# felipemcoelho/nf4-triton-dequantization

Hardware: AMD Instinct MI355X
Metric: dequantized elements/s (4096x4096 NF4->bf16, blocksize 64 / nested 256) (higher is better)
Workload: dtype f32

## Files before the change

nf4_triton_dequantization_amd/csrc/nf4_dequant.hip:

```cpp
#include <hip/hip_runtime.h>
#include <stdint.h>

#include "../../include/nf4_dequant.h"
#include "nf4_common.h"

namespace {

using namespace nf4dq;

enum Mode : int { kRef = 0, kSingle = 1, kBnb = 2, kBnbSingle = 3 };

struct Desc {
    const uint32_t* packed;
    const uint8_t* a1;
    const float* a2;
    const float* code2;
    u32x4* out;
    float offset;
    uint32_t nbytes;
    uint32_t tile_begin;
    uint32_t groups;
    FastDiv nb;
    FastDiv n2;
    FastDiv bpr;
    uint32_t blk_shift;
    uint32_t blk2_shift;
    uint32_t blk_base;
};

#ifndef NF4_FLAT_STAMPS
#define NF4_FLAT_STAMPS 0
#endif

template <int MAXB>
struct Batch {
    Desc d[MAXB];
    uint32_t count;
    uint32_t total_tiles;
#if NF4_FLAT_STAMPS
    unsigned long long* stamps;
#endif
};

#if NF4_FLAT_STAMPS
#define NF4_FSTAMP(slot_, val_)                                                                      \
    do {                                                                                             \
        __builtin_amdgcn_sched_barrier(0);                                                           \
        if (lane == 0) bt.stamps[(blockIdx.x * kFlatWaves + (threadIdx.x >> 6)) * 4u + (slot_)] = (val_); \
        __builtin_amdgcn_sched_barrier(0);                                                           \
    } while (0)
#define NF4_FNOW() __builtin_amdgcn_s_memrealtime()
#else
#define NF4_FSTAMP(slot_, val_) \
    do {                        \
    } while (0)
#define NF4_FNOW() 0ull
#endif

template <int DT>
__device__ __forceinline__ void store1(void* out, int64_t i, float x) {
    if constexpr (DT == NF4DQ_BF16) {
        reinterpret_cast<__bf16*>(out)[i] = (__bf16)x;
    } else if constexpr (DT == NF4DQ_F16) {
        reinterpret_cast<_Float16*>(out)[i] = (_Float16)opaque(x);
    } else {
        reinterpret_cast<float*>(out)[i] = x;
    }
}

#ifndef NF4_DQ_FLAT_WAVES
#define NF4_DQ_FLAT_WAVES 4
#endif
#ifndef NF4_DQ_U
#define NF4_DQ_U 4
#endif
#ifndef NF4_DQ_AUX_STORE
#define NF4_DQ_AUX_STORE 18
#endif
#ifndef NF4_DQ_AUX_LOAD
#define NF4_DQ_AUX_LOAD 2
#endif
#ifndef NF4_DQ_SCALE_FIRST
#define NF4_DQ_SCALE_FIRST 0
#endif
#ifndef NF4_DQ_SCALE_NT
#define NF4_DQ_SCALE_NT 0
#endif
#ifndef NF4_DQ_DECODE
#define NF4_DQ_DECODE 1
#endif
#ifndef NF4_DQ_SINGLE_FAST
#define NF4_DQ_SINGLE_FAST 1
#endif
#ifndef NF4_DQ_ABL_NOSCALE
#define NF4_DQ_ABL_NOSCALE 0
#endif



constexpr int kWg = 256;
constexpr int kFlatWaves = NF4_DQ_FLAT_WAVES;
constexpr int kFlatWg = 64 * kFlatWaves;
constexpr int kU = NF4_DQ_U;

constexpr int kAuxStore = NF4_DQ_AUX_STORE;
constexpr int kAuxLoad = NF4_DQ_AUX_LOAD;

template <int DT>
constexpr uint32_t out_bytes_per_packed_byte() { return DT == NF4DQ_F32 ? 8u : 4u; }
template <int DT>
constexpr uint32_t lane_bytes() { return DT == NF4DQ_F32 ? 2u : 4u; }
template <int DT>
constexpr uint32_t tile_bytes() { return 64u * lane_bytes<DT>() * kU; }

struct TileIn {
    uint32_t w[kU];
    uint32_t a1;
    float a2;
};

template <int DT>
__device__ __forceinline__ uint32_t tile_block(const Desc& D, uint32_t base, uint32_t lane) {
    constexpr uint32_t kTileBytes = tile_bytes<DT>();
    const uint32_t bsh = D.blk_shift;
    const uint32_t bpt = kTileBytes >> bsh;
    uint32_t g = (base >> bsh) + (bpt ? (lane & (bpt - 1u)) : 0u);
    const uint32_t nblk = (D.nbytes + (1u << bsh) - 1u) >> bsh;
    g = g < nblk ? g : nblk - 1u;
    return g + D.blk_base;
}

template <int DT, int MODE>
__device__ __forceinline__ TileIn tile_load(const Desc& D, __amdgpu_buffer_rsrc_t rp, uint32_t base, uint32_t lane) {
    constexpr uint32_t LB = lane_bytes<DT>();
    TileIn in;
    auto packed_loads = [&]() {
#pragma unroll
        for (int j = 0; j < kU; ++j) {
            const uint32_t off = base + 64u * LB * j + LB * lane;
            if constexpr (LB == 4) {
                in.w[j] = __builtin_amdgcn_raw_buffer_load_b32(rp, off, 0, kAuxLoad);
            } else {
                in.w[j] = __builtin_amdgcn_raw_buffer_load_b16(rp, off, 0, kAuxLoad);
            }
        }
    };
    if constexpr (!NF4_DQ_SCALE_FIRST) packed_loads();
    const uint32_t g = tile_block<DT>(D, base, lane);
    if constexpr (NF4_DQ_ABL_NOSCALE) {
        in.a1 = g & 255u;
        in.a2 = 0.01f;
    } else if constexpr (MODE == kRef) {
        const uint32_t r = fdiv(g, D.bpr);
        const uint32_t b = g - r * D.bpr.d;
        const uint8_t* pa1 = D.a1 + fmodu(g, D.nb);
        const float* pa2 = D.a2 + fmodu(r * D.groups + (b >> 2), D.n2);
        if constexpr (NF4_DQ_SCALE_NT) {
            in.a1 = __builtin_nontemporal_load(pa1);
            in.a2 = __builtin_nontemporal_load(pa2);
        } else {
            in.a1 = *pa1;
            in.a2 = *pa2;
        }
    } else if constexpr (MODE == kSingle) {
        const uint32_t r = fdiv(g, D.bpr);
        const uint32_t b = g - r * D.bpr.d;
        in.a2 = D.a2[r * D.n2.d + b];
    } else if constexpr (MODE == kBnb) {
        in.a1 = D.a1[g];
        in.a2 = D.a2[g >> D.blk2_shift];
    } else {
        in.a2 = D.a2[g];
    }
    if constexpr (NF4_DQ_SCALE_FIRST) packed_loads();
    return in;
}

template <int DT, int MODE>
__device__ __forceinline__ void tile_finish(const Desc& D, __amdgpu_buffer_rsrc_t ro, const float* lut,
                                            const TileIn& in, uint32_t base, uint32_t lane, const float* code2s) {
    float s;
    if constexpr (MODE == kRef) {
        s = ((float)in.a1 / 127.0f) * in.a2;
    } else if constexpr (MODE == kBnb) {
        s = code2s[in.a1] * in.a2 + D.offset;
    } else {
        s = in.a2;
    }
    const uint32_t bsh = D.blk_shift;
    constexpr uint32_t kOB = out_bytes_per_packed_byte<DT>();
    constexpr uint32_t LB = lane_bytes<DT>();
#pragma unroll
    for (int j = 0; j < kU; ++j) {
        const uint32_t rel = 64u * LB * j + LB * lane;
        const float sj = __shfl(s, (int)(rel >> bsh), 64);
        const uint32_t w = in.w[j];
        const uint32_t hi4 = (w >> 2) & 0x3C3C3C3Cu;
        const uint32_t lo4 = (w << 2) & 0x3C3C3C3Cu;
        const char* t = reinterpret_cast<const char*>(lut);
        float v[2 * LB];
#pragma unroll
        for (int k = 0; k < (int)LB; ++k) {
            v[2 * k] = *reinterpret_cast<const float*>(t + ((hi4 >> (8 * k)) & 0xFFu)) * sj;
            v[2 * k + 1] = *reinterpret_cast<const float*>(t + ((lo4 >> (8 * k)) & 0xFFu)) * sj;
        }
        const uint32_t ob = (base + rel) * kOB;
        if constexpr (DT == NF4DQ_F32) {
            u32x4 o = {__float_as_uint(v[0]), __float_as_uint(v[1]), __float_as_uint(v[2]), __float_as_uint(v[3])};
            __builtin_amdgcn_raw_buffer_store_b128(o, ro, ob, 0, kAuxStore);
        } else {
            u32x4 o = {pack2<DT>(v[0], v[1]), pack2<DT>(v[2], v[3]), pack2<DT>(v[4], v[5]), pack2<DT>(v[6], v[7])};
            __builtin_amdgcn_raw_buffer_store_b128(o, ro, ob, 0, kAuxStore);
        }
    }
}

typedef uint16_t __attribute__((may_alias)) u16_alias;
typedef uint32_t __attribute__((may_alias)) u32_alias;
typedef uint32_t u32x4_alias __attribute__((ext_vector_type(4), may_alias));

struct TblCtx {
    char* tbl;
    uint32_t tb;
    f32x2 c01;
};

template <int DT, int MODE>
__device__ __forceinline__ void tile_finish_tbl(const Desc& D, __amdgpu_buffer_rsrc_t ro, const TileIn& in,
                                                uint32_t base, uint32_t lane, const float* code2s,
                                                const TblCtx& c) {
    float s;
    if constexpr (MODE == kRef) {
        s = ((float)in.a1 / 127.0f) * in.a2;
    } else if constexpr (MODE == kBnb) {
        s = code2s[in.a1] * in.a2 + D.offset;
    } else {
        s = in.a2;
    }
    const uint32_t bsh = D.blk_shift;
    const uint32_t k = lane & 7u;
#pragma unroll
    for (int j = 0; j < kU; ++j) {
        const uint32_t rel = 256u * j + 4u * lane;
        const float sj = __shfl(s, (int)(rel >> bsh), 64);
        *reinterpret_cast<u32_alias*>(c.tbl + c.tb + 4u * k) = pack2<DT>(c.c01.x * sj, c.c01.y * sj);
        const uint32_t w = in.w[j];
        const uint32_t hb = (w >> 3) & 0x1E1E1E1Eu;
        const uint32_t lb = (w << 1) & 0x1E1E1E1Eu;
        uint32_t o[4];
#pragma unroll
        for (int b = 0; b < 4; ++b) {
            const uint32_t ah = __builtin_amdgcn_perm(hb, c.tb, 0x03020104u + b);
            const uint32_t al = __builtin_amdgcn_perm(lb, c.tb, 0x03020104u + b);
            const uint32_t vh = *reinterpret_cast<const u16_alias*>(c.tbl + ah);
            const uint32_t vl = *reinterpret_cast<const u16_alias*>(c.tbl + al);
            o[b] = vh | (vl << 16);
        }
        const u32x4 ov = {o[0], o[1], o[2], o[3]};
        __builtin_amdgcn_raw_buffer_store_b128(ov, ro, (base + rel) * 4u, 0, kAuxStore);
    }
}

template <int MAXB>
__device__ __forceinline__ uint32_t find_matrix(const Batch<MAXB>& bt, uint32_t t, uint32_t k) {
    if constexpr (MAXB > 1) {
        while (k + 1 < bt.count && t >= bt.d[k + 1].tile_begin) ++k;
    }
    return k;
}

struct Cursor {
    uint32_t t, k, base;
    bool valid;
};

template <int DT, int MAXB>
__device__ __forceinline__ Cursor cursor_at(const Batch<MAXB>& bt, uint32_t t, uint32_t k_hint) {
    constexpr uint32_t kTileBytes = tile_bytes<DT>();
    Cursor c;
    c.t = t;
    c.valid = t < bt.total_tiles;
    c.k = c.valid ? find_matrix(bt, t, k_hint) : k_hint;
    c.base = c.valid ? (t - bt.d[c.k].tile_begin) * kTileBytes : 0xFFFFF000u;
    return c;
}

template <int DT, int MAXB>
__device__ __forceinline__ void make_rsrcs(const Batch<MAXB>& bt, uint32_t k, __amdgpu_buffer_rsrc_t& rp,
                                           __amdgpu_buffer_rsrc_t& ro) {
    constexpr uint32_t kOB = out_bytes_per_packed_byte<DT>();
    rp = __builtin_amdgcn_make_buffer_rsrc((void*)bt.d[k].packed, 0, bt.d[k].nbytes, kRsrcFlags);
    ro = __builtin_amdgcn_make_buffer_rsrc((void*)bt.d[k].out, 0, bt.d[k].nbytes * kOB, kRsrcFlags);
}

template <int DT, int MODE, int MAXB>
__global__ __launch_bounds__(kFlatWg) void nf4_flat_kernel(const Batch<MAXB> bt) {
    __shared__ __attribute__((aligned(16))) float lut[16];
    __shared__ __attribute__((aligned(16))) float code2s[MODE == kBnb ? 256 : 1];
    constexpr bool kTbl = NF4_DQ_DECODE == 1 && DT != NF4DQ_F32;
    __shared__ __attribute__((aligned(256))) char tbl[kTbl ? kFlatWaves * 2048 : 4];
    const uint32_t lane = threadIdx.x & 63u;
#if NF4_FLAT_STAMPS
    const unsigned long long t_entry = NF4_FNOW();
    unsigned long long tiles_done = 0;
#endif
    const uint32_t t0 = __builtin_amdgcn_readfirstlane(blockIdx.x * kFlatWaves + (threadIdx.x >> 6));
    const uint32_t nwaves = gridDim.x * kFlatWaves;

    float c2w = 0.0f;
    if constexpr (MODE == kBnb) c2w = bt.d[0].code2[threadIdx.x & 255u];
    Cursor ca = cursor_at<DT>(bt, t0, 0u);
    __amdgpu_buffer_rsrc_t rpa, roa;
    make_rsrcs<DT>(bt, ca.k, rpa, roa);
    TileIn A = tile_load<DT, MODE>(bt.d[ca.k], rpa, ca.base, lane);
    const bool multi = !NF4_DQ_SINGLE_FAST || ca.t + nwaves < bt.total_tiles;
    if (multi) {
        const u32x4 z = {0u, 0u, 0u, 0u};
#pragma unroll
        for (int j = 0; j < kU; ++j) __builtin_amdgcn_raw_buffer_store_b128(z, roa, 0xFFFFF000u + 16u * j, 0, kAuxStore);
    }
    write_lut(lut);
    if constexpr (MODE == kBnb) {
        if constexpr (kFlatWg >= 256) {
            if (threadIdx.x < 256u) code2s[threadIdx.x] = c2w;
        } else {
            for (uint32_t i = threadIdx.x; i < 256u; i += kFlatWg) code2s[i] = bt.d[0].code2[i];
        }
    }
    __syncthreads();
    TblCtx tc{};
    if constexpr (kTbl) {
        tc.tbl = tbl;
        tc.tb = ((threadIdx.x >> 6) << 11) + ((lane >> 3) << 8);
        tc.c01 = *reinterpret_cast<const f32x2*>(lut + 2u * (lane & 7u));
    }
    if (!ca.valid) {
        NF4_FSTAMP(0, t_entry);
        NF4_FSTAMP(1, 0ull);
        NF4_FSTAMP(2, NF4_FNOW());
        NF4_FSTAMP(3, 0ull);
        return;
    }
    if (!multi) {
        if constexpr (kTbl) tile_finish_tbl<DT, MODE>(bt.d[ca.k], roa, A, ca.base, lane, code2s, tc);
        else tile_finish<DT, MODE>(bt.d[ca.k], roa, lut, A, ca.base, lane, code2s);
#if NF4_FLAT_STAMPS
        NF4_FSTAMP(1, NF4_FNOW());
        __builtin_amdgcn_s_waitcnt(0);
        NF4_FSTAMP(0, t_entry);
        NF4_FSTAMP(2, NF4_FNOW());
        NF4_FSTAMP(3, 1ull);
#endif
        return;
    }
    while (true) {
        const Cursor cb = cursor_at<DT>(bt, ca.t + nwaves, ca.k);
        __amdgpu_buffer_rsrc_t rpb = rpa, rob = roa;
        if (MAXB > 1 && cb.k != ca.k) make_rsrcs<DT>(bt, cb.k, rpb, rob);
        TileIn B = tile_load<DT, MODE>(bt.d[cb.k], rpb, cb.base, lane);
        if constexpr (kTbl) tile_finish_tbl<DT, MODE>(bt.d[ca.k], roa, A, ca.base, lane, code2s, tc);
        else tile_finish<DT, MODE>(bt.d[ca.k], roa, lut, A, ca.base, lane, code2s);
#if NF4_FLAT_STAMPS
        if (tiles_done == 0) NF4_FSTAMP(1, NF4_FNOW());
        ++tiles_done;
#endif
        if (!cb.valid) break;

        const Cursor cn = cursor_at<DT>(bt, cb.t + nwaves, cb.k);
        __amdgpu_buffer_rsrc_t rpn = rpb, ron = rob;
        if (MAXB > 1 && cn.k != cb.k) make_rsrcs<DT>(bt, cn.k, rpn, ron);
        A = tile_load<DT, MODE>(bt.d[cn.k], rpn, cn.base, lane);
        if constexpr (kTbl) tile_finish_tbl<DT, MODE>(bt.d[cb.k], rob, B, cb.base, lane, code2s, tc);
        else tile_finish<DT, MODE>(bt.d[cb.k], rob, lut, B, cb.base, lane, code2s);
#if NF4_FLAT_STAMPS
        ++tiles_done;
#endif
        if (!cn.valid) break;
        ca = cn;
        rpa = rpn;
        roa = ron;
    }
#if NF4_FLAT_STAMPS
    __builtin_amdgcn_s_waitcnt(0);
    NF4_FSTAMP(0, t_entry);
    NF4_FSTAMP(2, NF4_FNOW());
    NF4_FSTAMP(3, tiles_done);
#endif
}

struct RowsArgs {
    const uint8_t* packed;
    const uint8_t* a1;
    const float* a2;
    void* out;
    int64_t m, n, stride, cols_b;
    int64_t nb, n2, bpr, groups, rs;
};

template <int DT, int MODE>
__global__ __launch_bounds__(kWg) void nf4_rows_kernel(const RowsArgs A) {
    __shared__ __attribute__((aligned(16))) float lut[16];
    write_lut(lut);
    __syncthreads();
    const int64_t total = A.m * A.cols_b;
    for (int64_t i = (int64_t)blockIdx.x * kWg + threadIdx.x; i < total; i += (int64_t)gridDim.x * kWg) {
        const int64_t r = i / A.cols_b;
        const int64_t j = i - r * A.cols_b;
        const int64_t b = j >> 5;
        float s;
        if constexpr (MODE == kRef) {
            const float q = (float)A.a1[(r * A.bpr + b) % A.nb];
            s = (q / 127.0f) * A.a2[(r * A.groups + (b >> 2)) % A.n2];
        } else {
            s = A.a2[r * A.rs + b];
        }
        const uint32_t byte = A.packed[r * A.stride + j];
        const int64_t c = 2 * j;
        store1<DT>(A.out, r * A.n + c, lut[byte >> 4] * s);
        if (c + 1 < A.n) store1<DT>(A.out, r * A.n + c + 1, lut[byte & 15u] * s);
    }
}

struct ChunkArgs {
    const uint8_t* packed;
    const uint8_t* a1;
    const float* a2;
    void* out;
    uint64_t packed_len;
    uint64_t out_elems;
    uint32_t stride;
    uint32_t n;
    uint32_t chunks;
    FastDiv L;
    FastDiv bpr;
    uint32_t groups;
    FastDiv nb, n2;
    uint32_t rs;
};

constexpr uint32_t kDrop = 0xFFFFFFF0u;
constexpr int kAuxPiece = 0;
constexpr uint32_t kStageBytes = 4128;
constexpr uint32_t kStageDummy = 4112;

inline __device__ uint32_t range32(uint64_t v) { return v > 0x7FFFFFFFull ? 0x7FFFFFFFu : (uint32_t)v; }

inline __device__ uint32_t opaque_mul(uint32_t a, uint32_t b) {
    uint32_t r = a * b;
    asm("" : "+v"(r));
    return r;
}

template <int DT>
__device__ __forceinline__ void chunk_table_build(char* ctbl, uint32_t region, uint32_t lane, float sb) {
    uint32_t e[8];
#pragma unroll
    for (int k = 0; k < 8; ++k)
        e[k] = pack2<DT>(__uint_as_float(kNf4Bits[2 * k]) * sb, __uint_as_float(kNf4Bits[2 * k + 1]) * sb);
    u32x4_alias* dst = reinterpret_cast<u32x4_alias*>(ctbl + region + 32u * lane);
    dst[0] = u32x4{e[0], e[1], e[2], e[3]};
    dst[1] = u32x4{e[4], e[5], e[6], e[7]};
}

__device__ __forceinline__ void chunk_table_decode(const char* ctbl, uint32_t region, uint32_t w, uint32_t t,
                                                   uint32_t (&p)[4]) {
    t &= 63u;
    const uint32_t base = region + ((t >> 3) << 8);
    const uint32_t rep = __builtin_amdgcn_perm(0u, (t & 7u) << 5, 0x00000000u);
    const uint32_t hb = ((w >> 3) & 0x1E1E1E1Eu) | rep;
    const uint32_t lb = ((w << 1) & 0x1E1E1E1Eu) | rep;
#pragma unroll
    for (int b = 0; b < 4; ++b) {
        const uint32_t ah = __builtin_amdgcn_perm(hb, base, 0x03020104u + b);
        const uint32_t al = __builtin_amdgcn_perm(lb, base, 0x03020104u + b);
        const uint32_t vh = *reinterpret_cast<const u16_alias*>(ctbl + ah);
        const uint32_t vl = *reinterpret_cast<const u16_alias*>(ctbl + al);
        p[b] = vh | (vl << 16);
    }
}

template <int DT, int MODE>
__global__ __launch_bounds__(kWg) void nf4_chunk_dense_kernel(const ChunkArgs A) {
    __shared__ __attribute__((aligned(256))) char ctbl[4 * 2048];
    const uint32_t lane = threadIdx.x & 63u;
    const uint32_t cw = __builtin_amdgcn_readfirstlane((blockIdx.x * 4u + (threadIdx.x >> 6)) * 256u);
    const __amdgpu_buffer_rsrc_t rp =
        __builtin_amdgcn_make_buffer_rsrc((void*)A.packed, 0, (uint32_t)A.packed_len, kRsrcFlags);
    const __amdgpu_buffer_rsrc_t ro =
        __builtin_amdgcn_make_buffer_rsrc(A.out, 0, (uint32_t)(A.out_elems * 2u), kRsrcFlags);
    uint32_t w[4];
#pragma unroll
    for (int j = 0; j < 4; ++j)
        w[j] = __builtin_amdgcn_raw_buffer_load_b32(rp, 4u * (cw + 64u * j + lane), 0, kAuxLoad);
    __builtin_amdgcn_sched_barrier(0);
    const uint32_t cw0 = min(cw, A.chunks - 1u);
    const uint32_t r0 = fdiv(cw0, A.L);
    const uint32_t q0 = cw0 - r0 * A.L.d;
    const uint32_t cl = min(cw + 255u, A.chunks - 1u);
    const uint32_t rl = fdiv(cl, A.L);
    const uint32_t g0 = r0 * A.bpr.d + (q0 >> 3);
    const uint32_t gl = rl * A.bpr.d + ((cl - rl * A.L.d) >> 3);
    float sb;
    {
        const uint32_t g = min(g0 + lane, gl);
        const uint32_t r = fdiv(g, A.bpr);
        const uint32_t b = g - r * A.bpr.d;
        if constexpr (MODE == kRef) {
            const float q8 = (float)A.a1[fmodu(g, A.nb)];
            sb = (q8 / 127.0f) * A.a2[fmodu(opaque_mul(r, A.groups) + (b >> 2), A.n2)];
        } else {
            sb = A.a2[opaque_mul(r, A.rs) + b];
        }
    }
    uint32_t gsel[4];
    {
        uint32_t q = q0 + lane;
        const bool wrap = q >= A.L.d;
        q = wrap ? q - A.L.d : q;
        uint32_t gr = (wrap ? A.bpr.d : 0u) + r0 * A.bpr.d - g0;
#pragma unroll
        for (int j = 0; j < 4; ++j) {
            if (j) {
                q += 64u;
                const bool wj = q >= A.L.d;
                q = wj ? q - A.L.d : q;
                gr += wj ? A.bpr.d : 0u;
            }
            gsel[j] = gr + (q >> 3);
        }
    }
    const uint32_t region = (threadIdx.x >> 6) << 11;
    chunk_table_build<DT>(ctbl, region, lane, sb);
#pragma unroll
    for (int j = 0; j < 4; ++j) {
        uint32_t p[4];
        chunk_table_decode(ctbl, region, w[j], gsel[j], p);
        const u32x4 o = {p[0], p[1], p[2], p[3]};
        __builtin_amdgcn_raw_buffer_store_b128(o, ro, 16u * (cw + 64u * j + lane), 0, kAuxStore);
    }
// ... 421 lines not shown
        const uint32_t cu = (uint32_t)max(W.c[j], 0);
        const uint32_t tA = min(W.gr[j] + (cu >> 6), 59u);
        const uint32_t to_blk = 64u - (cu & 63u), to_end = A.n - cu;
        const uint32_t ib_in = to_blk < to_end ? min(to_blk, 8u) : 8u, ib_end = min(to_end, 8u);
        uint32_t es, os;
        piece_codes<1, RE, TRI>(W.lo[j], W.hi[j], W.b[j], W.c[j], ib_in, ib_end, tA & 3u, W.lo2[j], W.hi2[j],
                                W.nb[j], es, os);
        const uint32_t base = region + ((tA >> 2) << 8);
        uint32_t p[4];
#pragma unroll
        for (int b = 0; b < 4; ++b) {
            const uint32_t ve = *reinterpret_cast<const u16_alias*>(ptbl + __builtin_amdgcn_perm(es, base, 0x03020104u + b));
            const uint32_t vo = *reinterpret_cast<const u16_alias*>(ptbl + __builtin_amdgcn_perm(os, base, 0x03020104u + b));
            p[b] = __builtin_amdgcn_perm(vo, ve, 0x05040100u);
        }
        const uint32_t k = kw + 64u * (uint32_t)j + lane;
        const int32_t f = W.fw + 8 * (64 * j + (int32_t)lane);
        const bool whole = f >= 0 && (uint32_t)f + 8u <= A.elems;
        const u32x4 o = {p[0], p[1], p[2], p[3]};
        __builtin_amdgcn_raw_buffer_store_b128(o, ro, whole ? 16u * k : kDrop, 0, kAuxStore);
        if (!whole && f < (int32_t)A.elems && f + 8 > 0) {
            const __amdgpu_buffer_rsrc_t rsp =
                __builtin_amdgcn_make_buffer_rsrc(A.out, 0, 2u * A.elems, kRsrcFlags);
#pragma unroll
            for (int i = 0; i < 8; ++i) {
                uint32_t oe = 2u * (uint32_t)(f + i);
                asm("" : "+v"(oe));
                __builtin_amdgcn_raw_buffer_store_b16((uint16_t)(p[i >> 1] >> (16 * (i & 1))), rsp, oe, 0,
                                                      kAuxPiece);
            }
        }
    }
}

constexpr uint32_t kPiece32Tbl = 12 * 256;

template <int MODE, int RE, bool TRI>
__global__ __launch_bounds__(kWg) void nf4_piece32_kernel(const PieceArgs A) {
    __shared__ __attribute__((aligned(256))) char ptbl[4 * kPiece32Tbl];
    const uint32_t lane = threadIdx.x & 63u;
    const uint32_t kw = __builtin_amdgcn_readfirstlane((blockIdx.x * 4u + (threadIdx.x >> 6)) * 256u);
    PieceWave<4, RE> W;
    if (!piece_wave<4, RE>(A, kw, lane, W)) return;
    const float sb = piece_scale<MODE>(A, W.g0, W.gl, lane);
    const uint32_t region = (threadIdx.x >> 6) * kPiece32Tbl;
    if (lane < 24u) {
        u32x4 e[4];
#pragma unroll
        for (int k = 0; k < 4; ++k)
            e[k] = u32x4{__float_as_uint(__uint_as_float(kNf4Bits[4 * k]) * sb),
                         __float_as_uint(__uint_as_float(kNf4Bits[4 * k + 1]) * sb),
                         __float_as_uint(__uint_as_float(kNf4Bits[4 * k + 2]) * sb),
                         __float_as_uint(__uint_as_float(kNf4Bits[4 * k + 3]) * sb)};
        u32x4_alias* d0 = reinterpret_cast<u32x4_alias*>(ptbl + region + ((lane >> 1) << 8) + ((lane & 1u) << 6));
#pragma unroll
        for (int k = 0; k < 4; ++k) d0[k] = e[k];
        if (lane >= 2u) {
            u32x4_alias* d1 = reinterpret_cast<u32x4_alias*>(ptbl + region + ((lane >> 1) << 8) - 256u + 128u +
                                                            ((lane & 1u) << 6));
#pragma unroll
            for (int k = 0; k < 4; ++k) d1[k] = e[k];
        }
    }
    const __amdgpu_buffer_rsrc_t ro =
        __builtin_amdgcn_make_buffer_rsrc(A.line, 0, 4u * (A.sa + A.elems), kRsrcFlags);
#pragma unroll
    for (int j = 0; j < 4; ++j) {
        const uint32_t cu = (uint32_t)max(W.c[j], 0);
        const uint32_t tA = min(W.gr[j] + (cu >> 6), 21u);
        const uint32_t to_blk = 64u - (cu & 63u), to_end = A.n - cu;
        const uint32_t ib_in = to_blk < to_end ? min(to_blk, 4u) : 4u, ib_end = min(to_end, 4u);
        uint32_t es, os;
        piece_codes<2, RE, TRI>(W.lo[j], W.hi[j], W.b[j], W.c[j], ib_in, ib_end, tA & 1u, W.lo2[j], W.hi2[j],
                                W.nb[j], es, os);
        const uint32_t base = region + ((tA >> 1) << 8);
        uint32_t p[4];
#pragma unroll
        for (int b = 0; b < 2; ++b) {
            p[2 * b] = *reinterpret_cast<const uint32_t*>(ptbl + __builtin_amdgcn_perm(es, base, 0x03020104u + b));
            p[2 * b + 1] = *reinterpret_cast<const uint32_t*>(ptbl + __builtin_amdgcn_perm(os, base, 0x03020104u + b));
        }
        const uint32_t k = kw + 64u * (uint32_t)j + lane;
        const int32_t f = W.fw + 4 * (64 * j + (int32_t)lane);
        const bool whole = f >= 0 && (uint32_t)f + 4u <= A.elems;
        const u32x4 o = {p[0], p[1], p[2], p[3]};
        __builtin_amdgcn_raw_buffer_store_b128(o, ro, whole ? 16u * k : kDrop, 0, kAuxStore);
        if (!whole && f < (int32_t)A.elems && f + 4 > 0) {
            const __amdgpu_buffer_rsrc_t rsp =
                __builtin_amdgcn_make_buffer_rsrc(A.out, 0, 4u * A.elems, kRsrcFlags);
#pragma unroll
            for (int i = 0; i < 4; ++i) {
                uint32_t oe = 4u * (uint32_t)(f + i);
                asm("" : "+v"(oe));
                __builtin_amdgcn_raw_buffer_store_b32(p[i], rsp, oe, 0, kAuxPiece);
            }
        }
    }
}

struct BnbBytesArgs {
    const uint8_t* packed;
    const uint8_t* a1;
    const float* code2;
    const float* a2;
    void* out;
    float offset;
    int64_t numel;
    int32_t blk_shift_elems, blk2_shift;
    int32_t single;
};

template <int DT>
__global__ __launch_bounds__(kWg) void nf4_bnb_bytes_kernel(const BnbBytesArgs A) {
    __shared__ __attribute__((aligned(16))) float lut[16];
    write_lut(lut);
    __syncthreads();
    const int64_t nbytes = (A.numel + 1) / 2;
    for (int64_t i = (int64_t)blockIdx.x * kWg + threadIdx.x; i < nbytes; i += (int64_t)gridDim.x * kWg) {
        const int64_t e = 2 * i;
        const int64_t blk = e >> A.blk_shift_elems;
        const float s = A.single ? A.a2[blk] : A.code2[A.a1[blk]] * A.a2[blk >> A.blk2_shift] + A.offset;
        const uint32_t byte = A.packed[i];
        store1<DT>(A.out, e, lut[byte >> 4] * s);
        if (e + 1 < A.numel) store1<DT>(A.out, e + 1, lut[byte & 15u] * s);
    }
}

inline int hip_rc(hipError_t e) { return e == hipSuccess ? NF4DQ_OK : NF4DQ_ERR_HIP_BASE + (int)e; }

inline bool valid_dtype(int32_t d) { return d == NF4DQ_F16 || d == NF4DQ_BF16 || d == NF4DQ_F32; }

inline bool aligned(const void* p, uintptr_t a) { return (reinterpret_cast<uintptr_t>(p) & (a - 1)) == 0; }

inline int ilog2(uint64_t v) {
    int s = 0;
    while ((uint64_t(1) << s) < v) ++s;
    return s;
}

constexpr nf4_launch_cfg kDefaultCfg = {4, 0, 1, 0};

#if NF4_FLAT_STAMPS
unsigned long long* g_stamps = nullptr;
#endif

int cu_count() {
    int dev = 0, cus = 0;
    if (hipGetDevice(&dev) != hipSuccess) return 256;
    if (hipDeviceGetAttribute(&cus, hipDeviceAttributeMultiprocessorCount, dev) != hipSuccess || cus <= 0) return 256;
    return cus;
}

template <int DT, int MODE, int MAXB>
void launch_one(const Batch<MAXB>& b, uint64_t blocks, hipStream_t st) {
    hipLaunchKernelGGL((nf4_flat_kernel<DT, MODE, MAXB>), dim3((unsigned)blocks), dim3(kFlatWg), 0, st, b);
}

template <int MAXB>
int launch_flat_batch(const Batch<MAXB>& bt, int dtype, int mode, const nf4_launch_cfg& cfg, hipStream_t st) {
    if (bt.count == 0) return NF4DQ_OK;
    const uint32_t tb = 64u * (dtype == NF4DQ_F32 ? 2u : 4u) * kU;
    Batch<MAXB> b = bt;
    uint32_t acc = 0;
    for (uint32_t i = 0; i < b.count; ++i) {
        b.d[i].tile_begin = acc;
        acc += (b.d[i].nbytes + tb - 1u) / tb;
    }
    b.total_tiles = acc;
    if (acc == 0) return NF4DQ_OK;
    uint64_t blocks = (acc + kFlatWaves - 1) / kFlatWaves;
    if (cfg.blocks_per_cu > 0) {
        const uint64_t cap = (uint64_t)cfg.blocks_per_cu * (uint64_t)cu_count();
        if (blocks > cap) blocks = cap;
    }
#if NF4_FLAT_STAMPS
    b.stamps = g_stamps;
#endif
#define NF4_D(DT_)                                                              \
    do {                                                                        \
        switch (mode) {                                                         \
            case kRef: launch_one<DT_, kRef, MAXB>(b, blocks, st); break;       \
            case kSingle: launch_one<DT_, kSingle, MAXB>(b, blocks, st); break; \
            case kBnb: launch_one<DT_, kBnb, MAXB>(b, blocks, st); break;       \
            default: launch_one<DT_, kBnbSingle, MAXB>(b, blocks, st); break;   \
        }                                                                       \
    } while (0)
    if (dtype == NF4DQ_BF16) NF4_D(NF4DQ_BF16);
    else if (dtype == NF4DQ_F16) NF4_D(NF4DQ_F16);
    else NF4_D(NF4DQ_F32);
#undef NF4_D
    return hip_rc(hipGetLastError());
}

inline unsigned rows_grid(int64_t work) {
    int64_t b = (work + kWg - 1) / kWg;
    if (b > 65536) b = 65536;
    if (b < 1) b = 1;
    return (unsigned)b;
}

int check_common(const uint8_t* packed, int64_t packed_len, const void* out, int32_t dtype, int64_t m, int64_t n) {
    if (!valid_dtype(dtype)) return NF4DQ_ERR_ARG;
    if (m < 0 || n < 0 || packed_len < 0) return NF4DQ_ERR_ARG;
    if (m == 0 || n == 0) return NF4DQ_OK;
    if (!packed || !out) return NF4DQ_ERR_ARG;
    if (packed_len % m) return NF4DQ_ERR_SHAPE;
    if (packed_len / m < (n + 1) / 2) return NF4DQ_ERR_SHAPE;
    return NF4DQ_OK;
}

constexpr int64_t kPieceBytes = int64_t(1) << 29;
constexpr int64_t kMaxFlatBlocks = int64_t(1) << 31;

bool flat_eligible(const uint8_t* packed, int64_t packed_len, const void* out, int64_t m, int64_t n) {
    return n % 64 == 0 && packed_len == m * (n / 2) && n / 2 < kPieceBytes && packed_len / 32 < kMaxFlatBlocks &&
           aligned(packed, 4) && aligned(out, 16);
}

inline int64_t piece_rows(int64_t n) { return (kPieceBytes - 1) / (n / 2); }

template <int MAXB>
int append_pieces(Batch<MAXB>& b, const Desc& proto, int64_t m, int64_t n, int32_t dtype, int mode,
                  hipStream_t st) {
    const int64_t rows = piece_rows(n);
    const int64_t ob = dtype == NF4DQ_F32 ? 4 * n : 2 * n;
    for (int64_t r0 = 0; r0 < m; r0 += rows) {
        const int64_t r1 = r0 + rows < m ? r0 + rows : m;
        Desc d = proto;
        d.packed = reinterpret_cast<const uint32_t*>(reinterpret_cast<const uint8_t*>(proto.packed) + r0 * (n / 2));
        d.out = reinterpret_cast<u32x4*>(reinterpret_cast<uint8_t*>(proto.out) + r0 * ob);
        d.nbytes = (uint32_t)((r1 - r0) * (n / 2));
        d.blk_base = (uint32_t)(r0 * (n / 64));
        d.tile_begin = b.total_tiles;
        b.d[b.count++] = d;
        b.total_tiles += (d.nbytes + 1023u) / 1024u;
        if (b.count == (uint32_t)MAXB || b.total_tiles > (1u << 30)) {
            const int rc = launch_flat_batch(b, dtype, mode, kDefaultCfg, st);
            if (rc) return rc;
            b.count = 0;
            b.total_tiles = 0;
        }
    }
    return NF4DQ_OK;
}

int launch_flat_matrix(const Desc& proto, int64_t m, int64_t n, int32_t dtype, int mode, const nf4_launch_cfg& cfg,
                       hipStream_t st) {
    const int64_t packed_len = m * (n / 2);
    if (packed_len < kPieceBytes) {
        Batch<1> b{};
        b.d[0] = proto;
        b.d[0].nbytes = (uint32_t)packed_len;
        b.count = 1;
        b.total_tiles = (uint32_t)((packed_len + 1023) / 1024);
        return launch_flat_batch(b, dtype, mode, cfg, st);
    }
    Batch<NF4DQ_BATCH_MAX> b{};
    const int rc = append_pieces(b, proto, m, n, dtype, mode, st);
    if (rc || b.count == 0) return rc;
    return launch_flat_batch(b, dtype, mode, kDefaultCfg, st);
}

Desc ref_desc(const uint8_t* packed, int64_t packed_len, const uint8_t* a1, int64_t nb, const float* a2,
              int64_t n2, void* out, int64_t n) {
    Desc d{};
    d.packed = reinterpret_cast<const uint32_t*>(packed);
    d.a1 = a1;
    d.a2 = a2;
    d.out = reinterpret_cast<u32x4*>(out);
    d.nbytes = packed_len < kPieceBytes ? (uint32_t)packed_len : 0u;
    const int64_t bpr = (n + 63) / 64;
    d.groups = (uint32_t)((bpr + 3) / 4);
    d.nb = make_fastdiv((uint32_t)(nb > (int64_t(1) << 31) ? (int64_t(1) << 31) : nb));
    d.n2 = make_fastdiv((uint32_t)(n2 > (int64_t(1) << 31) ? (int64_t(1) << 31) : n2));
    d.bpr = make_fastdiv((uint32_t)bpr);
    d.blk_shift = 5;
    return d;
}

bool chunk_args(ChunkArgs& A, const uint8_t* packed, int64_t packed_len, void* out, int32_t dtype, int64_t m,
                int64_t n) {
    const int64_t stride = packed_len / m;
    const int64_t L = ((n + 1) / 2 + 3) / 4;
    const int64_t bpr = (n + 63) / 64;
    const int64_t ob = dtype == NF4DQ_F32 ? 4 : 2;
    const int64_t span = 256 / L + 2;
    const int64_t lim = int64_t(1) << 31;
    if (m * L >= lim - 1024 || m * bpr >= lim || n >= (int64_t(1) << 28) || span * stride >= lim ||
        span * n * ob >= lim || !aligned(out, (uintptr_t)ob))
        return false;
    A.packed = packed;
    A.out = out;
    A.packed_len = (uint64_t)packed_len;
    A.out_elems = (uint64_t)(m * n);
    A.stride = (uint32_t)stride;
    A.n = (uint32_t)n;
    A.chunks = (uint32_t)(m * L);
    A.L = make_fastdiv((uint32_t)L);
    A.bpr = make_fastdiv((uint32_t)bpr);
    A.groups = (uint32_t)((bpr + 3) / 4);
    return true;
}

template <int DT, int MODE, int LW>
void launch_chunks_lw(const ChunkArgs& A, int sw, unsigned g, hipStream_t st) {
    if (sw == 16) hipLaunchKernelGGL((nf4_chunk_kernel<DT, MODE, LW, 16>), dim3(g), dim3(kWg), 0, st, A);
    else hipLaunchKernelGGL((nf4_chunk_kernel<DT, MODE, LW, 4>), dim3(g), dim3(kWg), 0, st, A);
}

bool dense_eligible(const ChunkArgs& A, int32_t dtype) {
    return dtype != NF4DQ_F32 && A.L.d >= 64u && A.stride == 4u * A.L.d && A.n % 8u == 0 && aligned(A.packed, 4) &&
           aligned(A.out, 16) && A.chunks < (1u << 27);
}

bool piece_eligible(const ChunkArgs& A, int32_t dtype) {
    const uint64_t half = (A.n + 1u) / 2u;
    const uint64_t rows = A.out_elems / A.n;
    const uint64_t ob = dtype == NF4DQ_F32 ? 4u : 2u;
    if (A.stride != half && dtype != NF4DQ_F32 && A.n % 8u == 0 && aligned(A.out, 16)) return false;
    return A.stride >= half && A.packed_len == rows * A.stride && A.n >= 512u &&
           ob * (A.out_elems + 64u) < (uint64_t(1) << 31) && A.packed_len + 8u < (uint64_t(1) << 31);
}

template <int MODE, int DT, int RE, bool TRI>
void launch_pieces_k(const PieceArgs& P, unsigned g, hipStream_t st) {
    if constexpr (DT == NF4DQ_F32) hipLaunchKernelGGL((nf4_piece32_kernel<MODE, RE, TRI>), dim3(g), dim3(kWg), 0, st, P);
    else hipLaunchKernelGGL((nf4_piece_kernel<DT, MODE, RE, TRI>), dim3(g), dim3(kWg), 0, st, P);
}

template <int MODE, int DT, int RE>
void launch_pieces_re(const PieceArgs& P, unsigned g, hipStream_t st) {
    const uint32_t tail = P.n % 64u;
    if (tail != 0u && tail < (DT == NF4DQ_F32 ? 4u : 8u)) launch_pieces_k<MODE, DT, RE, true>(P, g, st);
    else launch_pieces_k<MODE, DT, RE, false>(P, g, st);
}

template <int MODE, int DT>
void launch_pieces_dt(const PieceArgs& P, unsigned g, hipStream_t st) {
// ... 301 lines not shown
```

Measured before the change: 2269 billion.

## Add single-tile-per-wave flat kernel with scalar args for uncapped single-tensor launches

Adds a specialized flat kernel used when there is one tensor and no per-CU block cap. Each wave handles exactly one tile, and the kernel takes scalar arguments instead of the large Batch struct, which drops the cursor loop, the prefetch pipeline and the dummy warm-up stores. A scheduling barrier after the packed loads keeps them issued ahead of the scale loads. The cost is that the software pipelining across tiles within a wave is lost, so each wave's latency is no longer hidden by its own next-tile loads.

```diff
diff --git a/nf4_triton_dequantization_amd/csrc/nf4_dequant.hip b/nf4_triton_dequantization_amd/csrc/nf4_dequant.hip
--- a/nf4_triton_dequantization_amd/csrc/nf4_dequant.hip
+++ b/nf4_triton_dequantization_amd/csrc/nf4_dequant.hip
@@ -46,7 +46,7 @@
 #define NF4_FSTAMP(slot_, val_)                                                                      \
     do {                                                                                             \
         __builtin_amdgcn_sched_barrier(0);                                                           \
-        if (lane == 0) bt.stamps[(blockIdx.x * kFlatWaves + (threadIdx.x >> 6)) * 4u + (slot_)] = (val_); \
+        if (lane == 0) stamps[(blockIdx.x * kFlatWaves + (threadIdx.x >> 6)) * 4u + (slot_)] = (val_);    \
         __builtin_amdgcn_sched_barrier(0);                                                           \
     } while (0)
 #define NF4_FNOW() __builtin_amdgcn_s_memrealtime()
@@ -68,6 +68,9 @@
     }
 }
 
+#ifndef NF4_DQ_FLAT1
+#define NF4_DQ_FLAT1 1
+#endif
 #ifndef NF4_DQ_FLAT_WAVES
 #define NF4_DQ_FLAT_WAVES 4
 #endif
@@ -130,7 +133,7 @@
     return g + D.blk_base;
 }
 
-template <int DT, int MODE>
+template <int DT, int MODE, bool FENCE = false>
 __device__ __forceinline__ TileIn tile_load(const Desc& D, __amdgpu_buffer_rsrc_t rp, uint32_t base, uint32_t lane) {
     constexpr uint32_t LB = lane_bytes<DT>();
     TileIn in;
@@ -145,7 +148,10 @@
             }
         }
     };
-    if constexpr (!NF4_DQ_SCALE_FIRST) packed_loads();
+    if constexpr (!NF4_DQ_SCALE_FIRST) {
+        packed_loads();
+        if constexpr (FENCE) __builtin_amdgcn_sched_barrier(0);
+    }
     const uint32_t g = tile_block<DT>(D, base, lane);
     if constexpr (NF4_DQ_ABL_NOSCALE) {
         in.a1 = g & 255u;
@@ -303,6 +309,7 @@
 #if NF4_FLAT_STAMPS
     const unsigned long long t_entry = NF4_FNOW();
     unsigned long long tiles_done = 0;
+    unsigned long long* const stamps = bt.stamps;
 #endif
     const uint32_t t0 = __builtin_amdgcn_readfirstlane(blockIdx.x * kFlatWaves + (threadIdx.x >> 6));
     const uint32_t nwaves = gridDim.x * kFlatWaves;
@@ -385,6 +392,77 @@
     NF4_FSTAMP(0, t_entry);
     NF4_FSTAMP(2, NF4_FNOW());
     NF4_FSTAMP(3, tiles_done);
+#endif
+}
+
+template <int DT, int MODE>
+__global__ __launch_bounds__(kFlatWg) void nf4_flat1_kernel(
+    const uint32_t* packed, uint32_t nbytes, uint32_t tiles, u32x4* out,
+    const uint8_t* a1, const float* a2, uint32_t blk_shift, uint32_t blk_base, uint32_t groups, uint32_t bpr_d,
+    uint32_t bpr_mul, uint32_t bpr_shift, uint32_t nb_d, uint32_t nb_mul, uint32_t nb_shift, uint32_t n2_d,
+    uint32_t n2_mul, uint32_t n2_shift, const float* code2, float offset, uint32_t blk2_shift
+#if NF4_FLAT_STAMPS
+    , unsigned long long* stamps
+#endif
+) {
+    __shared__ __attribute__((aligned(16))) float lut[16];
+    __shared__ __attribute__((aligned(16))) float code2s[MODE == kBnb ? 256 : 1];
+    constexpr bool kTbl = NF4_DQ_DECODE == 1 && DT != NF4DQ_F32;
+    __shared__ __attribute__((aligned(256))) char tbl[kTbl ? kFlatWaves * 2048 : 4];
+    const uint32_t lane = threadIdx.x & 63u;
+#if NF4_FLAT_STAMPS
+    const unsigned long long t_entry = NF4_FNOW();
+#endif
+    const uint32_t t0 = __builtin_amdgcn_readfirstlane(blockIdx.x * kFlatWaves + (threadIdx.x >> 6));
+    const bool valid = t0 < tiles;
+    const uint32_t base = valid ? t0 * tile_bytes<DT>() : 0xFFFFF000u;
+    Desc D;
+    D.packed = packed;
+    D.a1 = a1;
+    D.a2 = a2;
+    D.code2 = code2;
+    D.out = out;
+    D.offset = offset;
+    D.nbytes = nbytes;
+    D.tile_begin = 0u;
+    D.groups = groups;
+    D.nb = FastDiv{nb_d, nb_mul, nb_shift};
+    D.n2 = FastDiv{n2_d, n2_mul, n2_shift};
+    D.bpr = FastDiv{bpr_d, bpr_mul, bpr_shift};
+    D.blk_shift = blk_shift;
+    D.blk2_shift = blk2_shift;
+    D.blk_base = blk_base;
+    const __amdgpu_buffer_rsrc_t rp = __builtin_amdgcn_make_buffer_rsrc((void*)packed, 0, nbytes, kRsrcFlags);
+    const __amdgpu_buffer_rsrc_t ro =
+        __builtin_amdgcn_make_buffer_rsrc((void*)out, 0, nbytes * out_bytes_per_packed_byte<DT>(), kRsrcFlags);
+    const TileIn A = tile_load<DT, MODE, true>(D, rp, base, lane);
+    write_lut(lut);
+    if constexpr (MODE == kBnb) {
+        for (uint32_t i = threadIdx.x; i < 256u; i += kFlatWg) code2s[i] = code2[i];
+    }
+    __syncthreads();
+    if (!valid) {
+        NF4_FSTAMP(0, t_entry);
+        NF4_FSTAMP(1, 0ull);
+        NF4_FSTAMP(2, NF4_FNOW());
+        NF4_FSTAMP(3, 0ull);
+        return;
+    }
+    if constexpr (kTbl) {
+        TblCtx tc;
+        tc.tbl = tbl;
+        tc.tb = ((threadIdx.x >> 6) << 11) + ((lane >> 3) << 8);
+        tc.c01 = *reinterpret_cast<const f32x2*>(lut + 2u * (lane & 7u));
+        tile_finish_tbl<DT, MODE>(D, ro, A, base, lane, code2s, tc);
+    } else {
+        tile_finish<DT, MODE>(D, ro, lut, A, base, lane, code2s);
+    }
+#if NF4_FLAT_STAMPS
+    NF4_FSTAMP(1, NF4_FNOW());
+    __builtin_amdgcn_s_waitcnt(0);
+    NF4_FSTAMP(0, t_entry);
+    NF4_FSTAMP(2, NF4_FNOW());
+    NF4_FSTAMP(3, 1ull);
 #endif
 }
 
@@ -1112,7 +1190,21 @@
 }
 
 template <int DT, int MODE, int MAXB>
-void launch_one(const Batch<MAXB>& b, uint64_t blocks, hipStream_t st) {
+void launch_one(const Batch<MAXB>& b, uint64_t blocks, bool one_tile, hipStream_t st) {
+    if constexpr (MAXB == 1 && NF4_DQ_FLAT1) {
+        if (one_tile) {
+            const Desc& d = b.d[0];
+            nf4_flat1_kernel<DT, MODE><<<dim3((unsigned)blocks), dim3(kFlatWg), 0, st>>>(
+                d.packed, d.nbytes, b.total_tiles, d.out, d.a1, d.a2, d.blk_shift, d.blk_base, d.groups, d.bpr.d,
+                d.bpr.mul, d.bpr.shift, d.nb.d, d.nb.mul, d.nb.shift, d.n2.d, d.n2.mul, d.n2.shift, d.code2, d.offset,
+                d.blk2_shift
+#if NF4_FLAT_STAMPS
+                , b.stamps
+#endif
+            );
+            return;
+        }
+    }
     hipLaunchKernelGGL((nf4_flat_kernel<DT, MODE, MAXB>), dim3((unsigned)blocks), dim3(kFlatWg), 0, st, b);
 }
 
@@ -1129,6 +1221,7 @@
     b.total_tiles = acc;
     if (acc == 0) return NF4DQ_OK;
     uint64_t blocks = (acc + kFlatWaves - 1) / kFlatWaves;
+    const bool one_tile = cfg.blocks_per_cu <= 0;
     if (cfg.blocks_per_cu > 0) {
         const uint64_t cap = (uint64_t)cfg.blocks_per_cu * (uint64_t)cu_count();
         if (blocks > cap) blocks = cap;
@@ -1136,14 +1229,14 @@
 #if NF4_FLAT_STAMPS
     b.stamps = g_stamps;
 #endif
-#define NF4_D(DT_)                                                              \
-    do {                                                                        \
-        switch (mode) {                                                         \
-            case kRef: launch_one<DT_, kRef, MAXB>(b, blocks, st); break;       \
-            case kSingle: launch_one<DT_, kSingle, MAXB>(b, blocks, st); break; \
-            case kBnb: launch_one<DT_, kBnb, MAXB>(b, blocks, st); break;       \
-            default: launch_one<DT_, kBnbSingle, MAXB>(b, blocks, st); break;   \
-        }                                                                       \
+#define NF4_D(DT_)                                                                        \
+    do {                                                                                  \
+        switch (mode) {                                                                   \
+            case kRef: launch_one<DT_, kRef, MAXB>(b, blocks, one_tile, st); break;       \
+            case kSingle: launch_one<DT_, kSingle, MAXB>(b, blocks, one_tile, st); break; \
+            case kBnb: launch_one<DT_, kBnb, MAXB>(b, blocks, one_tile, st); break;       \
+            default: launch_one<DT_, kBnbSingle, MAXB>(b, blocks, one_tile, st); break;   \
+        }                                                                                 \
     } while (0)
     if (dtype == NF4DQ_BF16) NF4_D(NF4DQ_BF16);
     else if (dtype == NF4DQ_F16) NF4_D(NF4DQ_F16);
```

Result: faster. 2324 billion (median of 6 runs) (+2.4%).
